# Gadersd/whisper-burn

Measured on NVIDIA H100. Metric: audio-seconds/sec, higher is better.
Workload: dtype f32 (fp16-exact weights, fp32 activations/accumulate)

## Files before the change

whisper-burn_b200/csrc/decoder4.cu:

```cuda
#include <cooperative_groups.h>

#include "dec_common.cuh"

namespace cg = cooperative_groups;

namespace wb {

namespace {

#ifndef D4_ASYNC
#define D4_ASYNC 1
#endif
#define D4_EXCHANGE(IDX, RXBYTES, SEND, PF)                  \
    do {                                                     \
        WB_FINE();                                           \
        __syncthreads();                                     \
        WB_FINE();                                           \
        SEND();                                              \
        WB_FINE();                                           \
        if (D4_ASYNC) {                                      \
            PF();                                            \
            WB_FINE();                                       \
            xwait(xbar + (IDX), (RXBYTES), lc & 1u);         \
        } else {                                             \
            cluster_arrive();                                \
            PF();                                            \
            WB_FINE();                                       \
            cluster_wait();                                  \
        }                                                    \
    } while (0)
#ifndef D4_FINE
#define D4_FINE 0
#endif
#if D4_FINE
#define WB_FINE() WB_TRACE()
#else
#define WB_FINE() do { } while (0)
#endif

constexpr int CS = 16;
constexpr int LG_NBUF = 3;
constexpr int LG_RB = 8;
constexpr int KV_STG = 4;
#ifndef D4_L2_CKV_KEEP
#define D4_L2_CKV_KEEP 0
#endif
__device__ __forceinline__ uint64_t ckv_policy() { return D4_L2_CKV_KEEP ? l2_policy_evict_last() : l2_policy_evict_first(); }

__device__ __forceinline__ void cluster_arrive() { asm volatile("barrier.cluster.arrive.release.aligned;" ::: "memory"); }
__device__ __forceinline__ void cluster_wait() { asm volatile("barrier.cluster.wait.acquire.aligned;" ::: "memory"); }

template <int NR>
struct RowBias {
    float bias[NR];
    float bias_own;
};
template <int NR, int VPL>
struct RowRegs : RowBias<NR> {
    uint4 v[NR][VPL];
};

template <int NR>
__device__ __forceinline__ void load_bias(const float* __restrict__ bias, int row0, int step, RowBias<NR>& r) {
    const int lane = threadIdx.x & 31;
#pragma unroll
    for (int i = 0; i < NR; ++i) r.bias[i] = __ldg(bias + row0 + i * step);
    r.bias_own = __ldg(bias + row0 + min(lane >> 1, NR - 1) * step);
}
template <int NR, int VPL>
__device__ __forceinline__ void load_rows(const __half* __restrict__ W, const float* __restrict__ bias, int K, int row0, int step,
                                          RowRegs<NR, VPL>& r, uint64_t pol) {
    const int lane = threadIdx.x & 31, nv = K / 8;
    load_bias<NR>(bias, row0, step, r);
#pragma unroll
    for (int i = 0; i < NR; ++i) {
        const uint4* p = reinterpret_cast<const uint4*>(W + (int64_t)(row0 + i * step) * K);
#pragma unroll
        for (int j = 0; j < VPL; ++j) {
            const int v = j * 32 + lane;
            r.v[i][j] = v < nv ? ldg_l2(p + v, pol) : make_uint4(0, 0, 0, 0);
        }
    }
}
template <int NR>
__device__ __forceinline__ float warp_reduce_owner(const float (&acc)[NR]) {
    const int lane = threadIdx.x & 31;
    float v8[8], v4[4], v2[2];
    {
        const bool up = lane & 16;
#pragma unroll
        for (int i = 0; i < 8; ++i) {
            const float lo = i < NR ? acc[i] : 0.0f, hi = i + 8 < NR ? acc[i + 8] : 0.0f;
            const float recv = __shfl_xor_sync(0xffffffffu, up ? lo : hi, 16);
            v8[i] = (up ? hi : lo) + recv;
        }
    }
    {
        const bool up = lane & 8;
#pragma unroll
        for (int i = 0; i < 4; ++i) {
            const float recv = __shfl_xor_sync(0xffffffffu, up ? v8[i] : v8[i + 4], 8);
            v4[i] = (up ? v8[i + 4] : v8[i]) + recv;
        }
    }
    {
        const bool up = lane & 4;
#pragma unroll
        for (int i = 0; i < 2; ++i) {
            const float recv = __shfl_xor_sync(0xffffffffu, up ? v4[i] : v4[i + 2], 4);
            v2[i] = (up ? v4[i + 2] : v4[i]) + recv;
        }
    }
    const bool up = lane & 2;
    float v = (up ? v2[1] : v2[0]) + __shfl_xor_sync(0xffffffffu, up ? v2[0] : v2[1], 2);
    v += __shfl_xor_sync(0xffffffffu, v, 1);
    return v;
}

template <int NR, int VPL, bool REDUCE, typename WV>
__device__ __forceinline__ void dot_rows(WV&& wv, const float* xs, int K, float (&acc)[NR]) {
    const int lane = threadIdx.x & 31, nv = K / 8;
#pragma unroll
    for (int i = 0; i < NR; ++i) acc[i] = 0.0f;
#pragma unroll
    for (int j = 0; j < VPL; ++j) {
        const int v = j * 32 + lane;
        if (v < nv) {
            const float4 x0 = *reinterpret_cast<const float4*>(xs + v * 8);
            const float4 x1 = *reinterpret_cast<const float4*>(xs + v * 8 + 4);
#pragma unroll
            for (int i = 0; i < NR; ++i) {
                float w[8];
                cvt8(wv(i, j), w);
                float a = acc[i];
                a = fmaf(w[0], x0.x, a); a = fmaf(w[1], x0.y, a); a = fmaf(w[2], x0.z, a); a = fmaf(w[3], x0.w, a);
                a = fmaf(w[4], x1.x, a); a = fmaf(w[5], x1.y, a); a = fmaf(w[6], x1.z, a); a = fmaf(w[7], x1.w, a);
                acc[i] = a;
            }
        }
    }
    if constexpr (REDUCE) {
#pragma unroll
        for (int i = 0; i < NR; ++i) acc[i] = warp_sum(acc[i]);
    }
}
template <int NR, int VPL, bool REDUCE = true>
__device__ __forceinline__ void dot_rows1(const RowRegs<NR, VPL>& r, const float* xs, int K, float (&acc)[NR]) {
    dot_rows<NR, VPL, REDUCE>([&](int i, int j) { return r.v[i][j]; }, xs, K, acc);
}
template <int NR, int VPL, bool REDUCE = true>
__device__ __forceinline__ void dot_rows1s(const uint8_t* ws, const float* xs, int K, float (&acc)[NR]) {
    const int lane = threadIdx.x & 31, nv = K / 8;
    const uint4* w = reinterpret_cast<const uint4*>(ws) + (threadIdx.x >> 5) * nv;
    dot_rows<NR, VPL, REDUCE>([&](int i, int j) { return w[i * NW * nv + j * 32 + lane]; }, xs, K, acc);
}
__device__ __forceinline__ void bulk_rows(uint8_t* dst, const __half* W, int K, int row0, int n, uint64_t* bar) {
    const uint32_t bytes = (uint32_t)n * K * 2;
    fence_proxy_async();
    mbar_expect_tx(bar, bytes);
    bulk_g2s_l2(dst, W + (int64_t)row0 * K, bytes, bar, l2_policy_evict_last());
}

__device__ __forceinline__ void st_async_v4(uint32_t raddr, const float4& v, uint32_t rbar) {
    asm volatile("st.async.shared::cluster.mbarrier::complete_tx::bytes.v4.f32 [%0], {%1, %2, %3, %4}, [%5];" ::"r"(raddr), "f"(v.x),
                 "f"(v.y), "f"(v.z), "f"(v.w), "r"(rbar)
                 : "memory");
}
__device__ __forceinline__ void put16(cg::cluster_group& cl, float* dst, uint64_t* bar, int dest, const float4& v) {
#if D4_ASYNC
    st_async_v4(mapa_u32(smem_u32(dst), (uint32_t)dest), v, mapa_u32(smem_u32(bar), (uint32_t)dest));
#else
    *reinterpret_cast<float4*>(cl.map_shared_rank(dst, dest)) = v;
#endif
}
template <int CNT>
__device__ __forceinline__ void put_slice(cg::cluster_group& cl, const float* stage_s, float* dst_local, uint64_t* bar) {
    static_assert(CNT % 4 == 0, "slice must be a whole number of 16-byte vectors");
    constexpr int Q = CNT / 4;
    for (int i = threadIdx.x; i < CS * Q; i += NT) {
        const int dest = i / Q, q = i - dest * Q;
        put16(cl, dst_local + 4 * q, bar, dest, reinterpret_cast<const float4*>(stage_s)[q]);
    }
}
__device__ __forceinline__ void xwait(uint64_t* bar, uint32_t bytes, uint32_t parity) {
    if (threadIdx.x == 0) mbar_expect_tx(bar, bytes);
    const uint32_t mb = smem_u32(bar);
    uint32_t done = 0;
    int spins = 0;
    while (!done) {
        done = mbar_try_wait(mb, parity);
        if (!done && ++spins > (1 << 24)) __trap();
    }
}

template <int PF>
struct XRegs {
    float4 v[PF];
};
__device__ __forceinline__ float4 add4(const float4& a, const float4& b) {
    return make_float4(__fadd_rn(a.x, b.x), __fadd_rn(a.y, b.y), __fadd_rn(a.z, b.z), __fadd_rn(a.w, b.w));
}
template <int PF>
__device__ __forceinline__ void x_update(XRegs<PF>& x, const float* src_s, const float* d_s, float* dst_s) {
    const int lane = threadIdx.x & 31;
#pragma unroll
    for (int k = 0; k < PF; ++k)
        x.v[k] = add4(reinterpret_cast<const float4*>(src_s)[lane + 32 * k], reinterpret_cast<const float4*>(d_s)[lane + 32 * k]);
    if (dst_s != nullptr && threadIdx.x < 32) {
#pragma unroll
        for (int k = 0; k < PF; ++k) reinterpret_cast<float4*>(dst_s)[lane + 32 * k] = x.v[k];
    }
}
template <int D, int PF>
__device__ __forceinline__ void ln_fetch(float* lnp, const float* __restrict__ g, const float* __restrict__ b, uint64_t pol) {
    const int lane = threadIdx.x & 31;
#pragma unroll
    for (int k = 0; k < PF; ++k) {
        cp_async16_l2(lnp + 4 * (lane + 32 * k), g + 4 * (lane + 32 * k), pol);
        cp_async16_l2(lnp + D + 4 * (lane + 32 * k), b + 4 * (lane + 32 * k), pol);
    }
}
template <int D, int PF>
__device__ __forceinline__ void ln_warp(XRegs<PF>& x, const float* gb_s, float eps, int eps_outside, float* out_s) {
    const int lane = threadIdx.x & 31;
    cp_async_wait_all();
    float s = 0.0f;
#pragma unroll
    for (int k = 0; k < PF; ++k) s += (x.v[k].x + x.v[k].y) + (x.v[k].z + x.v[k].w);
    s = warp_sum(s);
    const float mean = __fdiv_rn(s, (float)D);
    float q = 0.0f;
#pragma unroll
    for (int k = 0; k < PF; ++k) {
        x.v[k].x = __fsub_rn(x.v[k].x, mean); x.v[k].y = __fsub_rn(x.v[k].y, mean);
        x.v[k].z = __fsub_rn(x.v[k].z, mean); x.v[k].w = __fsub_rn(x.v[k].w, mean);
        q = ln_sq_fma4(q, x.v[k]);
    }
    q = warp_sum(q);
    const float var = __fdiv_rn(q, (float)D);
    const float rinv = __fdiv_rn(1.0f, LN_DEN(var, eps, eps_outside));
#pragma unroll
    for (int k = 0; k < PF; ++k) {
        const float4 g = reinterpret_cast<const float4*>(gb_s)[lane + 32 * k];
        const float4 b = reinterpret_cast<const float4*>(gb_s + D)[lane + 32 * k];
        reinterpret_cast<float4*>(out_s)[lane + 32 * k] = ln_norm4_rcp(x.v[k], rinv, g, b);
    }
    __syncwarp();
}

template <int D, int RC, typename KVT>
__global__ void __launch_bounds__(NT, 1)
dec4_kernel(const DecArgs a) {
    extern __shared__ __align__(16) float sm[];
    cg::cluster_group cl = cg::this_cluster();
    constexpr int H = D / 64;
    constexpr int VPL = (D / 8 + 31) / 32;
    constexpr int VPL4 = (4 * D / 8 + 31) / 32;
    constexpr int NR_QKV = 3 * D / (CS * NW), NR_D = D / (CS * NW), NR_H = 4 * D / (CS * NW);
    const int L = a.L, V = a.V, R = a.R, t_max = a.t_max;
    const int tid = threadIdx.x, warp = tid >> 5, lane = tid & 31;
    const int rank = (int)cl.block_rank();
    const int row = blockIdx.x / CS;
    const bool active = row < R;

    float* lnp = sm + warp * 2 * D;
    float* qkv_s = sm + NW * 2 * D;
    float* att_s = qkv_s + 3 * D;
    float* dl_s = att_s + D;
    float* q2_s = dl_s + D;
    float* hid_s = q2_s + D;
    float* part_s = hid_s + 4 * D;
    float* wm = part_s + CS * 68;
    float* wl = wm + NW;
    float* wo = wl + NW;
    float* ao = wo + NW * 64;
    float* ML = ao + 64;
    constexpr int STG_N = 4 * D / CS > 68 ? 4 * D / CS : 68;
    float* stg_s = ML + 4;
    float* xb = stg_s + STG_N;
    float* xn_s = xb + 2 * D;
    float* red = xn_s + D;
    constexpr int RINGW = (LG_NBUF * LG_RB * D * 2 > KV_STG * 8 * 128 * 4) ? LG_NBUF * LG_RB * D * 2 : KV_STG * 8 * 128 * 4;
    constexpr int LG_PITCH = D * 2;
    uint8_t* ring = reinterpret_cast<uint8_t*>(red + NW * 4 * RC * 6);
    uint64_t* lg_bar = reinterpret_cast<uint64_t*>(ring + (size_t)NW * RINGW);
    uint64_t* kv_bar = lg_bar + NW * LG_NBUF;
    uint64_t* xbar = kv_bar + NW * KV_STG;
    uint64_t* wt_bar = xbar + 8;
    uint4* pl_hi = reinterpret_cast<uint4*>(wt_bar + 4);
    uint4* pl_lo = pl_hi + (D / 32) * 32;
    constexpr int QKV_B = 3 * D / CS * D * 2, W1_B = 4 * D / CS * D * 2, W2_B = D / CS * 4 * D * 2;
    constexpr int QKV_OFF = 0, W1_OFF = 0, W2_OFF = W1_OFF + W1_B;
    static_assert(W2_OFF + W2_B <= NW * RINGW, "W1 and W2 must fit the ring");
    static_assert(QKV_OFF + QKV_B <= W2_OFF, "the next layer's Wqkv arrives while W2 is read: no overlap");
    static_assert(QKV_B % 16 == 0 && W1_B % 16 == 0 && W2_B % 16 == 0 && W2_OFF % 16 == 0, "bulk copies move 16-byte units");
    if (lane == 0) {
        for (int j = 0; j < KV_STG; ++j) mbar_init(kv_bar + warp * KV_STG + j, 1);
        for (int j = 0; j < LG_NBUF; ++j) mbar_init(lg_bar + warp * LG_NBUF + j, 1);
        if (warp == 0) {
            for (int j = 0; j < 8; ++j) mbar_init(xbar + j, 1);
            for (int j = 0; j < 3; ++j) mbar_init(wt_bar + j, 1);
        }
        mbar_fence_init();
    }
    cl.sync();
    unsigned int lc = 0;
    unsigned int kv_count = 0;
    unsigned int lg_count = 0;
    unsigned int gen = 0;
    unsigned int lstep = 0;
    int tr_n = 0;
    const float scale = a.qk_scale;
    auto issue_qkv = [&](int l) {
        if (tid == 0) bulk_rows(ring + QKV_OFF, reinterpret_cast<const __half*>(a.layers[l].Wqkv), D, rank * (3 * D / CS), 3 * D / CS, wt_bar + 0);
    };
    auto demote = [&]() {
        const size_t gt = (size_t)blockIdx.x * NT + tid, gn = (size_t)gridDim.x * NT;
        for (int l = 0; l < L; ++l) {
            const DecLayer& W = a.layers[l];
            l2_demote(W.Wqkv, (size_t)3 * D * D * 2, gt, gn);
            l2_demote(W.Wo, (size_t)D * D * 2, gt, gn);
            l2_demote(W.Wcq, (size_t)D * D * 2, gt, gn);
            l2_demote(W.Wco, (size_t)D * D * 2, gt, gn);
            l2_demote(W.W1, (size_t)4 * D * D * 2, gt, gn);
            l2_demote(W.W2, (size_t)4 * D * D * 2, gt, gn);
            l2_demote(W.ln1_g, D * 4, gt, gn); l2_demote(W.ln1_b, D * 4, gt, gn); l2_demote(W.ln2_g, D * 4, gt, gn);
            l2_demote(W.ln2_b, D * 4, gt, gn); l2_demote(W.ln3_g, D * 4, gt, gn); l2_demote(W.ln3_b, D * 4, gt, gn);
        }
        l2_demote(a.lnf_g, D * 4, gt, gn);
        l2_demote(a.lnf_b, D * 4, gt, gn);
        const size_t kv_bytes = (size_t)L * a.Rmax * t_max * D * sizeof(KVT);
        l2_demote(a.kc, kv_bytes, gt, gn);
        l2_demote(a.vc, kv_bytes, gt, gn);
        if (D4_L2_CKV_KEEP) l2_demote(a.ckv, (size_t)L * a.Mcap * 2 * D * sizeof(KVT), gt, gn);
    };
    WB_TRACE();

    const __half* nullw = nullptr;
    (void)nullw;
    for (int step = 0; step < a.n_steps; ++step) {
        const int p = a.pos0 + step;
        const bool want_logits = p >= a.logits_from;
        constexpr int KH = D / 2, NCH = KH / 32;
        constexpr uint32_t BLKB = 16 * KH * 2;
        static_assert(LG_NBUF * LG_RB * D * 2 >= LG_NBUF * (int)BLKB, "ring slot too small");
        const __half* Et = reinterpret_cast<const __half*>(a.E_tiled);
        const int v_tiles = (V + 15) / 16;
        const int t0w = (int)blockIdx.x + (int)gridDim.x * warp, tstep = (int)gridDim.x * NW;
        const int my_tiles = t0w < v_tiles ? (v_tiles - t0w + tstep - 1) / tstep : 0;
        const int total = my_tiles * 2;
        auto tile_of = [&](int i) { return t0w + i * tstep; };
        uint8_t* wring = ring + (size_t)warp * RINGW;
        uint64_t* wbar = lg_bar + warp * LG_NBUF;
        auto issue = [&](int it) {
            if (it < total && lane == 0) {
                const int vt = tile_of(it >> 1);
                const int slot = (int)((lg_count + (unsigned int)it) % LG_NBUF);
                mbar_expect_tx(wbar + slot, BLKB);
                bulk_g2s_l2(wring + (size_t)slot * BLKB, Et + ((int64_t)vt * 2 + (it & 1)) * 16 * KH, BLKB, wbar + slot, l2_policy_evict_first());
            }
        };
        uint4* gpl_hi = reinterpret_cast<uint4*>(a.att_pl);
        uint4* gpl_lo = gpl_hi + (D / 32) * 32;
        if (want_logits && !active) {
#pragma unroll
            for (int j = 0; j < LG_NBUF; ++j) issue(j);
        }
        if (active) {
            const int tok = __ldcg(a.tokens + (int64_t)row * t_max + p);
            const int xh = rank % H, xci = rank / H;
            const int xnch = (CS - xh + H - 1) / H;
            const int xw = __ldcg(a.row_window + row);
            const int xT = a.win_T[xw];
            const int64_t xoff = a.win_row_off[xw] * (int64_t)(2 * D) + (int64_t)xh * xT * 128;
            const int sub = lane >> 2, l4 = lane & 3;
            const bool self_fast = p + 1 <= NW * 16;
            constexpr int PF = D / 128;
            static_assert(D % 128 == 0, "row must be a whole number of float4s per lane");
            int xsel = 0;
            XRegs<PF> x;
#pragma unroll
            for (int k = 0; k < PF; ++k)
                x.v[k] = add4(__ldg(reinterpret_cast<const float4*>(a.tok_emb + (int64_t)tok * D) + lane + 32 * k),
                              __ldg(reinterpret_cast<const float4*>(a.pos_emb + (int64_t)p * D) + lane + 32 * k));
            if (warp == 0) {
#pragma unroll
                for (int k = 0; k < PF; ++k) reinterpret_cast<float4*>(xb)[lane + 32 * k] = x.v[k];
            }
            RowBias<NR_QKV> b_qkv;
            load_bias<NR_QKV>(a.layers[0].bqkv, rank * (3 * D / CS) + warp, NW, b_qkv);
            if (step == 0) issue_qkv(0);
            if (step == 0) ln_fetch<D, PF>(lnp, a.layers[0].ln1_g, a.layers[0].ln1_b, l2_policy_evict_last());
            __syncthreads();
            for (int l = 0; l < L; ++l) {
                const DecLayer& W = a.layers[l];
                KVT* kcl = reinterpret_cast<KVT*>(a.kc) + (size_t)l * a.Rmax * t_max * D;
                KVT* vcl = reinterpret_cast<KVT*>(a.vc) + (size_t)l * a.Rmax * t_max * D;
                if (l > 0) {
                    x_update<PF>(x, xb + xsel * D, dl_s, xb + (xsel ^ 1) * D);
                    xsel ^= 1;
                }
                ln_warp<D, PF>(x, lnp, W.ln1_eps, a.eps_outside, xn_s);
                ln_fetch<D, PF>(lnp, W.ln2_g, W.ln2_b, l2_policy_evict_last());
                {
                    float acc[NR_QKV];
                    mbar_wait(wt_bar + 0, lc & 1u);
                    dot_rows1s<NR_QKV, VPL, false>(ring + QKV_OFF, xn_s, D, acc);
                    float mine = warp_reduce_owner<NR_QKV>(acc);
                    mine = __fadd_rn(mine, b_qkv.bias_own);
                    const int j = warp + (lane >> 1) * NW;
                    if (rank * (3 * D / CS) + j < 2 * D) mine = __fmul_rn(mine, scale);
                    if (!(lane & 1) && (lane >> 1) < NR_QKV) stg_s[j] = mine;
                }
                RowRegs<NR_D, VPL> w_o;
                constexpr int SNV = sizeof(KVT) == 4 ? 4 : 2;
                uint8_t* sring = ring + (size_t)warp * RINGW;
                auto pre_s2 = [&]() {
                    load_rows<NR_D, VPL>(reinterpret_cast<const __half*>(W.Wo), W.bo, D, rank * (D / CS) + warp, NW, w_o, l2_policy_evict_last());
                    if (rank < H && self_fast) {
#pragma unroll
                        for (int u = 0; u < 2; ++u) {
                            const int j = warp + NW * (u * 8 + sub);
                            if (j < p) {
                                const int64_t o = ((int64_t)row * t_max + j) * D + rank * 64 + l4 * 16;
#pragma unroll
                                for (int c = 0; c < SNV; ++c) {
                                    cp_async16_l2(sring + ((u * 2 + 0) * 4 + c) * 512 + lane * 16, reinterpret_cast<const uint4*>(kcl + o) + c, l2_policy_evict_last());
                                    cp_async16_l2(sring + ((u * 2 + 1) * 4 + c) * 512 + lane * 16, reinterpret_cast<const uint4*>(vcl + o) + c, l2_policy_evict_last());
                                }
                            }
                        }
                    }
                };
                auto send_s1 = [&]() {
                    put_slice<3 * D / CS>(cl, stg_s, qkv_s + rank * (3 * D / CS), xbar + 0);
                    if (tid < 3 * D / CS) {
                        const int n = rank * (3 * D / CS) + tid;
                        const float v = stg_s[tid];
                        if (n >= 2 * D) vcl[((int64_t)row * t_max + p) * D + (n - 2 * D)] = (KVT)v;
                        else if (n >= D) kcl[((int64_t)row * t_max + p) * D + (n - D)] = (KVT)v;
                    }
                };
                D4_EXCHANGE(0, 3 * D * 4, send_s1, pre_s2);
                if (D4_ASYNC && !self_fast) cl.sync();
                WB_TRACE();
                if (rank < H) {
                    const int h = rank;
                    if (self_fast) {
                        cp_async_wait_all();
                        float q[16];
#pragma unroll
                        for (int c = 0; c < 4; ++c) {
                            const float4 t4 = *reinterpret_cast<const float4*>(qkv_s + h * 64 + l4 * 16 + c * 4);
                            q[c * 4] = t4.x; q[c * 4 + 1] = t4.y; q[c * 4 + 2] = t4.z; q[c * 4 + 3] = t4.w;
                        }
                        AttnAcc A;
                        A.m = -INFINITY;
                        A.l = 0.0f;
#pragma unroll
                        for (int c = 0; c < 16; ++c) A.o[c] = 0.0f;
#pragma unroll
                        for (int u = 0; u < 2; ++u) {
                            const int j = warp + NW * (u * 8 + sub);
                            float4 skk[4], svv[4];
                            if (j < p) {
                                if constexpr (sizeof(KVT) == 4) {
#pragma unroll
                                    for (int c = 0; c < 4; ++c) {
                                        skk[c] = *reinterpret_cast<const float4*>(sring + ((u * 2 + 0) * 4 + c) * 512 + lane * 16);
                                        svv[c] = *reinterpret_cast<const float4*>(sring + ((u * 2 + 1) * 4 + c) * 512 + lane * 16);
                                    }
                                } else {
#pragma unroll
                                    for (int c = 0; c < 2; ++c) {
                                        float w8[8];
                                        cvt8(*reinterpret_cast<const uint4*>(sring + ((u * 2 + 0) * 4 + c) * 512 + lane * 16), w8);
                                        skk[2 * c] = make_float4(w8[0], w8[1], w8[2], w8[3]); skk[2 * c + 1] = make_float4(w8[4], w8[5], w8[6], w8[7]);
                                        cvt8(*reinterpret_cast<const uint4*>(sring + ((u * 2 + 1) * 4 + c) * 512 + lane * 16), w8);
                                        svv[2 * c] = make_float4(w8[0], w8[1], w8[2], w8[3]); svv[2 * c + 1] = make_float4(w8[4], w8[5], w8[6], w8[7]);
                                    }
                                }
                            } else {
#pragma unroll
                                for (int c = 0; c < 4; ++c) { skk[c] = make_float4(0.f, 0.f, 0.f, 0.f); svv[c] = skk[c]; }
                            }
                            if (j == p) {
#pragma unroll
                                for (int c = 0; c < 4; ++c) {
                                    float4 k4 = *reinterpret_cast<const float4*>(qkv_s + D + h * 64 + l4 * 16 + c * 4);
                                    float4 v4 = *reinterpret_cast<const float4*>(qkv_s + 2 * D + h * 64 + l4 * 16 + c * 4);
                                    if constexpr (sizeof(KVT) == 2) {
                                        k4 = make_float4((float)(KVT)k4.x, (float)(KVT)k4.y, (float)(KVT)k4.z, (float)(KVT)k4.w);
                                        v4 = make_float4((float)(KVT)v4.x, (float)(KVT)v4.y, (float)(KVT)v4.z, (float)(KVT)v4.w);
                                    }
                                    skk[c] = k4;
                                    svv[c] = v4;
                                }
                            }
                            attn_regs_step(q, skk, svv, j <= p, A);
                        }
                        attn_merge_subs(A);
                        attn_cta_tail(A, wm, wl, wo, ao, ML);
                    } else {
                        const KVT* kb = kcl + h * 64;
                        const KVT* vb = vcl + h * 64;
                        auto kp = [&](int j) { return kb + ((int64_t)row * t_max + j) * D; };
                        auto vp = [&](int j) { return vb + ((int64_t)row * t_max + j) * D; };
                        attn_cta(qkv_s + h * 64, p + 1, kp, vp, wm, wl, wo, ao, ML);
                    }
                }
                auto send_s2 = [&]() {
                    if (rank < H) {
                        const int dest = tid >> 4, q = tid & 15;
                        const float4 o4 = reinterpret_cast<const float4*>(ao)[q];
                        const float den = ML[1];
                        put16(cl, att_s + rank * 64 + 4 * q, xbar + 1, dest,
                              make_float4(__fdiv_rn(o4.x, den), __fdiv_rn(o4.y, den), __fdiv_rn(o4.z, den), __fdiv_rn(o4.w, den)));
                    }
                };
                auto pf_none = [&]() {};
                D4_EXCHANGE(1, D * 4, send_s2, pf_none);
                WB_TRACE();
                {
                    float acc[NR_D];
                    dot_rows1<NR_D, VPL>(w_o, att_s, D, acc);
                    WB_FINE();
                    if (lane == 0) {
#pragma unroll
                        for (int i = 0; i < NR_D; ++i) stg_s[warp + i * NW] = __fadd_rn(acc[i], w_o.bias[i]);
                    }
                }
                RowRegs<NR_D, VPL> w_cq;
                auto pre_s4 = [&]() {
                    load_rows<NR_D, VPL>(reinterpret_cast<const __half*>(W.Wcq), W.bcq, D, rank * (D / CS) + warp, NW, w_cq, l2_policy_evict_last());
                    fence_proxy_async();
                    attn_bulk_prefill<KV_STG, KVT, true>(reinterpret_cast<const KVT*>(a.ckv) + (size_t)l * a.Mcap * 2 * D + xoff, xT, xci * NW + warp,
                                                         xnch * NW, ring + (size_t)warp * RINGW, kv_bar + warp * KV_STG, kv_count, ckv_policy());
                };
                auto send_s3 = [&]() { put_slice<D / CS>(cl, stg_s, dl_s + rank * (D / CS), xbar + 2); };
                D4_EXCHANGE(2, D * 4, send_s3, pre_s4);
                WB_TRACE();
                x_update<PF>(x, xb + xsel * D, dl_s, xb + (xsel ^ 1) * D);
                xsel ^= 1;
                ln_warp<D, PF>(x, lnp, W.ln2_eps, a.eps_outside, xn_s);
                ln_fetch<D, PF>(lnp, W.ln3_g, W.ln3_b, l2_policy_evict_last());
                WB_FINE();
                {
                    float acc[NR_D];
                    dot_rows1<NR_D, VPL>(w_cq, xn_s, D, acc);
                    WB_FINE();
                    if (lane == 0) {
#pragma unroll
                        for (int i = 0; i < NR_D; ++i) stg_s[warp + i * NW] = __fmul_rn(__fadd_rn(acc[i], w_cq.bias[i]), scale);
                    }
                }
                RowRegs<NR_D, VPL> w_co;
                auto pre_s6 = [&]() { load_rows<NR_D, VPL>(reinterpret_cast<const __half*>(W.Wco), W.bco, D, rank * (D / CS) + warp, NW, w_co, l2_policy_evict_last()); };
                auto send_s4 = [&]() { put_slice<D / CS>(cl, stg_s, q2_s + rank * (D / CS), xbar + 3); };
                D4_EXCHANGE(3, D * 4, send_s4, pre_s6);
                WB_TRACE();
                {
                    const int h = xh, ci = xci, nch = xnch, T = xT;
                    const KVT* kbase = reinterpret_cast<const KVT*>(a.ckv) + (size_t)l * a.Mcap * 2 * D + xoff;
                    AttnAcc A;
                    attn_warp_bulk<KV_STG, KVT, true>(q2_s + h * 64, kbase, T, ci * NW + warp, nch * NW, 0, ring + (size_t)warp * RINGW,
                                                      kv_bar + warp * KV_STG, kv_count, A, true, ckv_policy());
                    if (lane < 4) {
#pragma unroll
                        for (int c = 0; c < 16; ++c) wo[warp * 64 + attn_bulk_dim<KVT>(lane, c)] = A.o[c];
                    }
                    if (lane == 0) { wm[warp] = A.m; wl[warp] = A.l; }
                    __syncthreads();
                    if (tid < 64) {
                        float M = -INFINITY;
#pragma unroll
                        for (int w2 = 0; w2 < NW; ++w2) M = fmaxf(M, wm[w2]);
                        float Ls = 0.0f, o = 0.0f;
#pragma unroll
                        for (int w2 = 0; w2 < NW; ++w2) {
                            const float m = wm[w2];
                            const float sc = m > -INFINITY ? expf(m - M) : 0.0f;
                            Ls += sc * wl[w2];
                            o += sc * wo[w2 * 64 + tid];
                        }
                        stg_s[4 + tid] = o;
                        if (tid < 4) stg_s[tid] = tid == 0 ? M : tid == 1 ? Ls : 0.0f;
                    }
                }
                auto send_s5 = [&]() { put_slice<68>(cl, stg_s, part_s + rank * 68, xbar + 4); };
                auto pre_mlp = [&]() {
                    if (tid == 0) {
                        bulk_rows(ring + W1_OFF, reinterpret_cast<const __half*>(W.W1), D, rank * (4 * D / CS), 4 * D / CS, wt_bar + 1);
                        bulk_rows(ring + W2_OFF, reinterpret_cast<const __half*>(W.W2), 4 * D, rank * (D / CS), D / CS, wt_bar + 2);
                    }
                };
                D4_EXCHANGE(4, CS * 68 * 4, send_s5, pre_mlp);
                WB_TRACE();
                for (int c = tid; c < D; c += NT) {
                    const int h = c / 64;
                    float M = -INFINITY;
                    for (int k = h; k < CS; k += H) M = fmaxf(M, part_s[k * 68]);
                    float den = 0.0f, num = 0.0f;
                    for (int k = h; k < CS; k += H) {
                        const float m = part_s[k * 68];
                        const float wgt = m > -INFINITY ? expf(m - M) : 0.0f;
                        den += wgt * part_s[k * 68 + 1];
                        num += wgt * part_s[k * 68 + 4 + (c & 63)];
                    }
                    att_s[c] = __fdiv_rn(num, den);
                }
                __syncthreads();
                {
                    float acc[NR_D];
                    dot_rows1<NR_D, VPL>(w_co, att_s, D, acc);
                    if (lane == 0) {
#pragma unroll
                        for (int i = 0; i < NR_D; ++i) stg_s[warp + i * NW] = __fadd_rn(acc[i], w_co.bias[i]);
                    }
                }
                RowBias<NR_H> b_1;
                auto pre_s7 = [&]() { load_bias<NR_H>(W.b1, rank * (4 * D / CS) + warp, NW, b_1); };
                auto send_s6 = [&]() { put_slice<D / CS>(cl, stg_s, dl_s + rank * (D / CS), xbar + 5); };
                D4_EXCHANGE(5, D * 4, send_s6, pre_s7);
                WB_TRACE();
                x_update<PF>(x, xb + xsel * D, dl_s, xb + (xsel ^ 1) * D);
                xsel ^= 1;
                ln_warp<D, PF>(x, lnp, W.ln3_eps, a.eps_outside, xn_s);
                if (l == L - 1 && want_logits && rank == 0 && warp == 0) {
                    ln_fetch<D, PF>(lnp, a.lnf_g, a.lnf_b, l2_policy_evict_last());
                } else {
                    const DecLayer& Wn = a.layers[l + 1 < L ? l + 1 : 0];
                    ln_fetch<D, PF>(lnp, Wn.ln1_g, Wn.ln1_b, l2_policy_evict_last());
                }
                WB_FINE();
                {
                    float acc[NR_H];
                    mbar_wait(wt_bar + 1, lc & 1u);
                    dot_rows1s<NR_H, VPL, false>(ring + W1_OFF, xn_s, D, acc);
                    float mine = warp_reduce_owner<NR_H>(acc);
                    mine = gelu_erf(__fadd_rn(mine, b_1.bias_own));
                    WB_FINE();
                    if (!(lane & 1) && (lane >> 1) < NR_H) stg_s[warp + (lane >> 1) * NW] = mine;
                }
                RowBias<NR_D> b_2;
                auto pre_s8 = [&]() {
                    load_bias<NR_D>(W.b2, rank * (D / CS) + warp, NW, b_2);
                    if (l + 1 < L) issue_qkv(l + 1);
                    else if (!want_logits && step + 1 < a.n_steps) issue_qkv(0);
                };
                auto send_s7 = [&]() { put_slice<4 * D / CS>(cl, stg_s, hid_s + rank * (4 * D / CS), xbar + 6); };
                D4_EXCHANGE(6, 4 * D * 4, send_s7, pre_s8);
                WB_TRACE();
                {
                    float acc[NR_D];
                    mbar_wait(wt_bar + 2, lc & 1u);
                    dot_rows1s<NR_D, VPL4>(ring + W2_OFF, hid_s, 4 * D, acc);
                    if (lane == 0) {
#pragma unroll
                        for (int i = 0; i < NR_D; ++i) stg_s[warp + i * NW] = __fadd_rn(acc[i], b_2.bias[i]);
                    }
                }
                auto pre_s1 = [&]() {
                    if (l + 1 < L) {
                        load_bias<NR_QKV>(a.layers[l + 1].bqkv, rank * (3 * D / CS) + warp, NW, b_qkv);
                    } else if (want_logits) {
                        fence_proxy_async();
#pragma unroll
                        for (int j = 0; j < LG_NBUF; ++j) issue(j);
                    }
                };
                auto send_s8 = [&]() { put_slice<D / CS>(cl, stg_s, dl_s + rank * (D / CS), xbar + 7); };
                D4_EXCHANGE(7, D * 4, send_s8, pre_s1);
                ++lc;
                WB_TRACE();
            }
            if (want_logits && rank == 0 && warp == 0) {
                x_update<PF>(x, xb + xsel * D, dl_s, nullptr);
                ln_warp<D, PF>(x, lnp, a.lnf_eps, a.eps_outside, xn_s);
#pragma unroll
                for (int k = 0; k < PF; ++k)
                    store_frag(gpl_hi, RC == 4 ? gpl_hi + 16 : gpl_lo, D / 32, row, 4 * (lane + 32 * k), reinterpret_cast<const float4*>(xn_s)[lane + 32 * k]);
                ln_fetch<D, PF>(lnp, a.layers[0].ln1_g, a.layers[0].ln1_b, l2_policy_evict_last());
            }
        }
        if (!want_logits) {
            if (D4_ASYNC && active) cl.sync();
            continue;
        }
        WB_TRACE();
        grid_sync(a.bar, gen);
        WB_TRACE();
        {
            const bool use_mask = SPECIAL_MASKED(a, p);
            const int eot_cap = a.loop_rules ? a.eot : -1;
            for (int i = tid; i < 2 * (D / 32) * 32; i += NT) cp_async16(pl_hi + i, gpl_hi + i);
            cp_async_wait_all();
            __syncthreads();
            WB_TRACE();
            const int g = lane >> 2, t = lane & 3;
            float m_run[2] = {-INFINITY, -INFINITY}, s_run[2] = {0.0f, 0.0f}, bv[2] = {-INFINITY, -INFINITY};
            int bi[2] = {INT_MAX, INT_MAX};
            float ah[4], al[4];
            unsigned int sp01 = 0;
#pragma unroll 1
            for (int it = 0; it < total; ++it) {
                const unsigned int cnt = lg_count + (unsigned int)it;
                const int slot = (int)(cnt % LG_NBUF);
                mbar_wait(wbar + slot, (cnt / LG_NBUF) & 1);
                const uint8_t* blk = wring + (size_t)slot * BLKB;
                const int half = it & 1;
                if (half == 0) {
#pragma unroll
                    for (int c = 0; c < 4; ++c) { ah[c] = 0.0f; al[c] = 0.0f; }
                    if (use_mask) {
                        const int n = tile_of(it >> 1) * 16 + g;
                        sp01 = (n < V ? ldg_l2(a.is_special + n, l2_policy_evict_first()) : 0u) | (n + 8 < V ? ldg_l2(a.is_special + n + 8, l2_policy_evict_first()) << 8 : 0u);
                    }
                }
#pragma unroll
                for (int c = 0; c < NCH; ++c) {
                    const uint4 a0 = *reinterpret_cast<const uint4*>(blk + (size_t)g * (KH * 2) + c * 64 + t * 16);
                    const uint4 a8 = *reinterpret_cast<const uint4*>(blk + (size_t)(g + 8) * (KH * 2) + c * 64 + t * 16);
                    const int chunk = half * NCH + c;
                    const uint4 bh = pl_hi[chunk * 32 + lane];
                    mma16816(ah, a0.x, a8.x, a0.y, a8.y, bh.x, bh.y);
                    mma16816(ah, a0.z, a8.z, a0.w, a8.w, bh.z, bh.w);
                    if constexpr (RC != 4) {
                        const uint4 bl = pl_lo[chunk * 32 + lane];
                        mma16816(al, a0.x, a8.x, a0.y, a8.y, bl.x, bl.y);
                        mma16816(al, a0.z, a8.z, a0.w, a8.w, bl.z, bl.w);
                    }
                }
                if (half == 1) {
                    const int n0 = tile_of(it >> 1) * 16;
#pragma unroll
                    for (int c = 0; c < 4; ++c) {
                        const int n = n0 + g + (c >> 1) * 8, e = c & 1;
                        if constexpr (RC == 4) al[c] = __shfl_xor_sync(0xffffffffu, ah[c], 2);
                        if (n < V && 2 * t + e < R) {
                            const float raw = hl_join(ah[c], al[c]);
                            const float v = (use_mask && ((sp01 >> ((c >> 1) * 8)) & 0xffu)) ? __fadd_rn(raw, -INFINITY) : raw;
                            if (v > -INFINITY) softmax_add(m_run[e], s_run[e], v);
                            if (cand_better(v, n, bv[e], bi[e])) { bv[e] = v; bi[e] = n; }
                            if (n == eot_cap) a.eot_logit[2 * t + e] = v;
                        }
                    }
                }
                __syncwarp();
                issue(it + LG_NBUF);
            }
            lg_count += (unsigned int)total;
            WB_TRACE();
#pragma unroll
            for (int e = 0; e < 2; ++e) {
#pragma unroll
                for (int off = 4; off < 32; off <<= 1) {
                    softmax_merge(m_run[e], s_run[e], __shfl_xor_sync(0xffffffffu, m_run[e], off), __shfl_xor_sync(0xffffffffu, s_run[e], off));
                    cand_xor(bv[e], bi[e], off);
                }
                if (g == 0) {
                    float* rec = red + (warp * 8 + 2 * t + e) * 4;
                    rec[0] = m_run[e]; rec[1] = s_run[e]; rec[2] = bv[e]; rec[3] = __int_as_float(bi[e]);
                }
            }
            __syncthreads();
            if (active && step + 1 < a.n_steps) issue_qkv(0);
            if (tid < R) fold_records_top1(a, red + tid * 4, NW, 8 * 4, (int64_t)blockIdx.x * R + tid);
        }
        WB_TRACE();
        ++lstep;
        __syncthreads();
        if (tid == 0) reinterpret_cast<int*>(ML)[2] = last_ticket(a.bar, lstep);
        __syncthreads();
        WB_TRACE();
        if (reinterpret_cast<int*>(ML)[2]) {
            __threadfence();
            for (int r = warp; r < R; r += NW) finish_row_top1<4>(a, r, p, gridDim.x);
            __syncthreads();
            if (tid == 0) release_flag(a.bar, lstep);
        }
        WB_TRACE();
        if (tid == 0) wait_flag(a.bar, lstep, 40000000000LL);
        __syncthreads();
        WB_TRACE();
        if (rows_open(a) == 0) {
            if (active && tid == 0 && step + 1 < a.n_steps) mbar_wait(wt_bar + 0, lc & 1u);
            if (blockIdx.x == 0 && tid == 0) decode_done(a, p + 1, 0, step + 1);
            demote();
            return;
        }
    }
    if (a.n_steps > 0 && a.pos0 + a.n_steps - 1 < a.logits_from) grid_sync(a.bar, gen);
    demote();
    if (blockIdx.x == 0 && tid == 0) decode_done(a, a.pos0 + a.n_steps, rows_open(a), a.n_steps);
}

template <int D, int RC>
constexpr size_t dec4_smem() {
    return sizeof(float) * ((size_t)(2 * NW + 13) * D + (4 * D / CS > 68 ? 4 * D / CS : 68) + CS * 68 + 2 * NW + NW * 64 + 64 + 4 + (size_t)NW * 4 * RC * 6 + 16) +
           (size_t)NW * std::max(LG_NBUF * LG_RB * D * 2, KV_STG * 8 * 128 * 4) + NW * LG_NBUF * 8 + NW * KV_STG * 8 + 8 * 8 + 4 * 8 + (size_t)2 * (D / 32) * 32 * 16 + 16;
}
static_assert(dec4_smem<384, 8>() <= 227 * 1024 && dec4_smem<384, 4>() <= 227 * 1024, "dec4_kernel exceeds the shared memory of an sm_90 CTA");

template <int D, int RC, typename KVT>
bool launch4_t(const DecArgs& a, cudaStream_t st) {
    const void* k = (const void*)dec4_kernel<D, RC, KVT>;
    const size_t smem = dec4_smem<D, RC>();
    static ClusterLaunch cl;
    const int n_cl = std::min(cl.capacity(k, CS, NT, smem, "dec4"), 8);
    if (n_cl < 1 || a.R > n_cl) return false;
    void* args[] = {(void*)&a};
    cl.launch(k, CS, n_cl, NT, smem, args, st, "dec4");
    return true;
}

}

bool launch_dec4(const DecArgs& a, bool w_half, cudaStream_t st) {
    if (!w_half || a.R > 8 || a.R < 1 || a.k != 1 || !a.greedy || a.use_cur_tok || a.anc != nullptr || a.logits_out != nullptr) return false;
    if (a.H * 64 != a.d || a.H > CS || a.E_tiled == nullptr) return false;
#define WB_D4(DD)                                                                                         \
    do {                                                                                                  \
        if (a.kv_half) return a.R <= 4 ? launch4_t<DD, 4, __half>(a, st) : launch4_t<DD, 8, __half>(a, st); \
        return a.R <= 4 ? launch4_t<DD, 4, float>(a, st) : launch4_t<DD, 8, float>(a, st);                 \
    } while (0)
    if (a.d == 384) WB_D4(384);
    if (a.d == 128) WB_D4(128);
#undef WB_D4
    return false;
}

}
```

Baseline: 2626.

## Bulk-copy biases with weights, issue MLP weights earlier, prefetch next token

Bias vectors for QKV, W1 and W2 are now loaded into shared memory by the same bulk async copies that bring in the weight tiles, replacing per-warp register bias loads scattered through the exchange prefetch hooks. The W1/W2 bulk copies are issued right after the attention merge barrier rather than inside the exchange. The next step's token is read early, and the finished-row check becomes a block-wide syncthreads_count. This is meant to cut global load latency on the critical path and free registers, at the cost of extra shared memory and reliance on the mbarrier transaction byte counts staying correct.

```diff
diff --git a/whisper-burn_b200/csrc/decoder4.cu b/whisper-burn_b200/csrc/decoder4.cu
--- a/whisper-burn_b200/csrc/decoder4.cu
+++ b/whisper-burn_b200/csrc/decoder4.cu
@@ -50,28 +50,18 @@
 __device__ __forceinline__ void cluster_arrive() { asm volatile("barrier.cluster.arrive.release.aligned;" ::: "memory"); }
 __device__ __forceinline__ void cluster_wait() { asm volatile("barrier.cluster.wait.acquire.aligned;" ::: "memory"); }
 
-template <int NR>
-struct RowBias {
+template <int NR, int VPL>
+struct RowRegs {
     float bias[NR];
-    float bias_own;
-};
-template <int NR, int VPL>
-struct RowRegs : RowBias<NR> {
     uint4 v[NR][VPL];
 };
 
-template <int NR>
-__device__ __forceinline__ void load_bias(const float* __restrict__ bias, int row0, int step, RowBias<NR>& r) {
-    const int lane = threadIdx.x & 31;
-#pragma unroll
-    for (int i = 0; i < NR; ++i) r.bias[i] = __ldg(bias + row0 + i * step);
-    r.bias_own = __ldg(bias + row0 + min(lane >> 1, NR - 1) * step);
-}
 template <int NR, int VPL>
 __device__ __forceinline__ void load_rows(const __half* __restrict__ W, const float* __restrict__ bias, int K, int row0, int step,
                                           RowRegs<NR, VPL>& r, uint64_t pol) {
     const int lane = threadIdx.x & 31, nv = K / 8;
-    load_bias<NR>(bias, row0, step, r);
+#pragma unroll
+    for (int i = 0; i < NR; ++i) r.bias[i] = __ldg(bias + row0 + i * step);
 #pragma unroll
     for (int i = 0; i < NR; ++i) {
         const uint4* p = reinterpret_cast<const uint4*>(W + (int64_t)(row0 + i * step) * K);
@@ -154,11 +144,12 @@
     const uint4* w = reinterpret_cast<const uint4*>(ws) + (threadIdx.x >> 5) * nv;
     dot_rows<NR, VPL, REDUCE>([&](int i, int j) { return w[i * NW * nv + j * 32 + lane]; }, xs, K, acc);
 }
-__device__ __forceinline__ void bulk_rows(uint8_t* dst, const __half* W, int K, int row0, int n, uint64_t* bar) {
+__device__ __forceinline__ void bulk_rows(uint8_t* dst, const __half* W, int K, int row0, int n, float* bdst, const float* bias, uint64_t* bar) {
     const uint32_t bytes = (uint32_t)n * K * 2;
     fence_proxy_async();
-    mbar_expect_tx(bar, bytes);
+    mbar_expect_tx(bar, bytes + (uint32_t)n * 4);
     bulk_g2s_l2(dst, W + (int64_t)row0 * K, bytes, bar, l2_policy_evict_last());
+    bulk_g2s(bdst, bias + row0, (uint32_t)n * 4, bar);
 }
 
 __device__ __forceinline__ void st_async_v4(uint32_t raddr, const float4& v, uint32_t rbar) {
@@ -289,11 +280,15 @@
     uint64_t* wt_bar = xbar + 8;
     uint4* pl_hi = reinterpret_cast<uint4*>(wt_bar + 4);
     uint4* pl_lo = pl_hi + (D / 32) * 32;
+    float* bqkv_s = reinterpret_cast<float*>(pl_lo + (D / 32) * 32);
+    float* b1_s = bqkv_s + 3 * D / CS;
+    float* b2_s = b1_s + 4 * D / CS;
     constexpr int QKV_B = 3 * D / CS * D * 2, W1_B = 4 * D / CS * D * 2, W2_B = D / CS * 4 * D * 2;
     constexpr int QKV_OFF = 0, W1_OFF = 0, W2_OFF = W1_OFF + W1_B;
     static_assert(W2_OFF + W2_B <= NW * RINGW, "W1 and W2 must fit the ring");
     static_assert(QKV_OFF + QKV_B <= W2_OFF, "the next layer's Wqkv arrives while W2 is read: no overlap");
-    static_assert(QKV_B % 16 == 0 && W1_B % 16 == 0 && W2_B % 16 == 0 && W2_OFF % 16 == 0, "bulk copies move 16-byte units");
+    static_assert(QKV_B % 16 == 0 && W1_B % 16 == 0 && W2_B % 16 == 0 && W2_OFF % 16 == 0 && (D / CS * 4) % 16 == 0,
+                  "bulk copies move 16-byte units");
     if (lane == 0) {
         for (int j = 0; j < KV_STG; ++j) mbar_init(kv_bar + warp * KV_STG + j, 1);
         for (int j = 0; j < LG_NBUF; ++j) mbar_init(lg_bar + warp * LG_NBUF + j, 1);
@@ -309,10 +304,13 @@
     unsigned int lg_count = 0;
     unsigned int gen = 0;
     unsigned int lstep = 0;
+    int tok_next = -1;
     int tr_n = 0;
     const float scale = a.qk_scale;
     auto issue_qkv = [&](int l) {
-        if (tid == 0) bulk_rows(ring + QKV_OFF, reinterpret_cast<const __half*>(a.layers[l].Wqkv), D, rank * (3 * D / CS), 3 * D / CS, wt_bar + 0);
+        if (tid == 0)
+            bulk_rows(ring + QKV_OFF, reinterpret_cast<const __half*>(a.layers[l].Wqkv), D, rank * (3 * D / CS), 3 * D / CS, bqkv_s, a.layers[l].bqkv,
+                      wt_bar + 0);
     };
     auto demote = [&]() {
         const size_t gt = (size_t)blockIdx.x * NT + tid, gn = (size_t)gridDim.x * NT;
@@ -367,7 +365,8 @@
             for (int j = 0; j < LG_NBUF; ++j) issue(j);
         }
         if (active) {
-            const int tok = __ldcg(a.tokens + (int64_t)row * t_max + p);
+            const int tok = tok_next >= 0 ? tok_next : __ldcg(a.tokens + (int64_t)row * t_max + p);
+            tok_next = -1;
             const int xh = rank % H, xci = rank / H;
             const int xnch = (CS - xh + H - 1) / H;
             const int xw = __ldcg(a.row_window + row);
@@ -387,8 +386,6 @@
 #pragma unroll
                 for (int k = 0; k < PF; ++k) reinterpret_cast<float4*>(xb)[lane + 32 * k] = x.v[k];
             }
-            RowBias<NR_QKV> b_qkv;
-            load_bias<NR_QKV>(a.layers[0].bqkv, rank * (3 * D / CS) + warp, NW, b_qkv);
             if (step == 0) issue_qkv(0);
             if (step == 0) ln_fetch<D, PF>(lnp, a.layers[0].ln1_g, a.layers[0].ln1_b, l2_policy_evict_last());
             __syncthreads();
@@ -407,7 +404,7 @@
                     mbar_wait(wt_bar + 0, lc & 1u);
                     dot_rows1s<NR_QKV, VPL, false>(ring + QKV_OFF, xn_s, D, acc);
                     float mine = warp_reduce_owner<NR_QKV>(acc);
-                    mine = __fadd_rn(mine, b_qkv.bias_own);
+                    mine = __fadd_rn(mine, bqkv_s[warp + min(lane >> 1, NR_QKV - 1) * NW]);
                     const int j = warp + (lane >> 1) * NW;
                     if (rank * (3 * D / CS) + j < 2 * D) mine = __fmul_rn(mine, scale);
                     if (!(lane & 1) && (lane >> 1) < NR_QKV) stg_s[j] = mine;
@@ -571,6 +568,10 @@
                     }
                     if (lane == 0) { wm[warp] = A.m; wl[warp] = A.l; }
                     __syncthreads();
+                    if (tid == 64) {
+                        bulk_rows(ring + W1_OFF, reinterpret_cast<const __half*>(W.W1), D, rank * (4 * D / CS), 4 * D / CS, b1_s, W.b1, wt_bar + 1);
+                        bulk_rows(ring + W2_OFF, reinterpret_cast<const __half*>(W.W2), 4 * D, rank * (D / CS), D / CS, b2_s, W.b2, wt_bar + 2);
+                    }
                     if (tid < 64) {
                         float M = -INFINITY;
 #pragma unroll
@@ -588,13 +589,7 @@
                     }
                 }
                 auto send_s5 = [&]() { put_slice<68>(cl, stg_s, part_s + rank * 68, xbar + 4); };
-                auto pre_mlp = [&]() {
-                    if (tid == 0) {
-                        bulk_rows(ring + W1_OFF, reinterpret_cast<const __half*>(W.W1), D, rank * (4 * D / CS), 4 * D / CS, wt_bar + 1);
-                        bulk_rows(ring + W2_OFF, reinterpret_cast<const __half*>(W.W2), 4 * D, rank * (D / CS), D / CS, wt_bar + 2);
-                    }
-                };
-                D4_EXCHANGE(4, CS * 68 * 4, send_s5, pre_mlp);
+                D4_EXCHANGE(4, CS * 68 * 4, send_s5, pf_none);
                 WB_TRACE();
                 for (int c = tid; c < D; c += NT) {
                     const int h = c / 64;
@@ -618,10 +613,8 @@
                         for (int i = 0; i < NR_D; ++i) stg_s[warp + i * NW] = __fadd_rn(acc[i], w_co.bias[i]);
                     }
                 }
-                RowBias<NR_H> b_1;
-                auto pre_s7 = [&]() { load_bias<NR_H>(W.b1, rank * (4 * D / CS) + warp, NW, b_1); };
                 auto send_s6 = [&]() { put_slice<D / CS>(cl, stg_s, dl_s + rank * (D / CS), xbar + 5); };
-                D4_EXCHANGE(5, D * 4, send_s6, pre_s7);
+                D4_EXCHANGE(5, D * 4, send_s6, pf_none);
                 WB_TRACE();
                 x_update<PF>(x, xb + xsel * D, dl_s, xb + (xsel ^ 1) * D);
                 xsel ^= 1;
@@ -638,13 +631,11 @@
                     mbar_wait(wt_bar + 1, lc & 1u);
                     dot_rows1s<NR_H, VPL, false>(ring + W1_OFF, xn_s, D, acc);
                     float mine = warp_reduce_owner<NR_H>(acc);
-                    mine = gelu_erf(__fadd_rn(mine, b_1.bias_own));
+                    mine = gelu_erf(__fadd_rn(mine, b1_s[warp + min(lane >> 1, NR_H - 1) * NW]));
                     WB_FINE();
                     if (!(lane & 1) && (lane >> 1) < NR_H) stg_s[warp + (lane >> 1) * NW] = mine;
                 }
-                RowBias<NR_D> b_2;
                 auto pre_s8 = [&]() {
-                    load_bias<NR_D>(W.b2, rank * (D / CS) + warp, NW, b_2);
                     if (l + 1 < L) issue_qkv(l + 1);
                     else if (!want_logits && step + 1 < a.n_steps) issue_qkv(0);
                 };
@@ -657,13 +648,11 @@
                     dot_rows1s<NR_D, VPL4>(ring + W2_OFF, hid_s, 4 * D, acc);
                     if (lane == 0) {
 #pragma unroll
-                        for (int i = 0; i < NR_D; ++i) stg_s[warp + i * NW] = __fadd_rn(acc[i], b_2.bias[i]);
+                        for (int i = 0; i < NR_D; ++i) stg_s[warp + i * NW] = __fadd_rn(acc[i], b2_s[warp + i * NW]);
                     }
                 }
                 auto pre_s1 = [&]() {
-                    if (l + 1 < L) {
-                        load_bias<NR_QKV>(a.layers[l + 1].bqkv, rank * (3 * D / CS) + warp, NW, b_qkv);
-                    } else if (want_logits) {
+                    if (l + 1 == L && want_logits) {
                         fence_proxy_async();
 #pragma unroll
                         for (int j = 0; j < LG_NBUF; ++j) issue(j);
@@ -783,7 +772,8 @@
         if (tid == 0) wait_flag(a.bar, lstep, 40000000000LL);
         __syncthreads();
         WB_TRACE();
-        if (rows_open(a) == 0) {
+        if (active && step + 1 < a.n_steps) tok_next = __ldcg(a.tokens + (int64_t)row * t_max + p + 1);
+        if (__syncthreads_count(tid < R && !(a.greedy && __ldcg(a.finished + tid))) == 0) {
             if (active && tid == 0 && step + 1 < a.n_steps) mbar_wait(wt_bar + 0, lc & 1u);
             if (blockIdx.x == 0 && tid == 0) decode_done(a, p + 1, 0, step + 1);
             demote();
@@ -798,7 +788,8 @@
 template <int D, int RC>
 constexpr size_t dec4_smem() {
     return sizeof(float) * ((size_t)(2 * NW + 13) * D + (4 * D / CS > 68 ? 4 * D / CS : 68) + CS * 68 + 2 * NW + NW * 64 + 64 + 4 + (size_t)NW * 4 * RC * 6 + 16) +
-           (size_t)NW * std::max(LG_NBUF * LG_RB * D * 2, KV_STG * 8 * 128 * 4) + NW * LG_NBUF * 8 + NW * KV_STG * 8 + 8 * 8 + 4 * 8 + (size_t)2 * (D / 32) * 32 * 16 + 16;
+           (size_t)NW * std::max(LG_NBUF * LG_RB * D * 2, KV_STG * 8 * 128 * 4) + NW * LG_NBUF * 8 + NW * KV_STG * 8 + 8 * 8 + 4 * 8 +
+           (size_t)2 * (D / 32) * 32 * 16 + sizeof(float) * (8 * D / CS) + 16;
 }
 static_assert(dec4_smem<384, 8>() <= 227 * 1024 && dec4_smem<384, 4>() <= 227 * 1024, "dec4_kernel exceeds the shared memory of an sm_90 CTA");
 
```

Measured after the change: 2689, median of 6. 1.02x the previous value.
